# MikeIvanichev/norma

Hardware: AMD Instinct MI355X
Metric: audio-sec/wall-sec (xRT) distil-large-v3 fp16 b32 (higher is better)
Workload: dtype f16

## Files before the change

include/norma_hip.h:

```cpp
#ifndef NORMA_HIP_H
#define NORMA_HIP_H

#include <stddef.h>
#include <stdint.h>

#ifdef __cplusplus
extern "C" {
#endif

#define NH_OK 0
#define NH_ERR_INVALID 1
#define NH_ERR_HIP 2
#define NH_ERR_STATE 3
#define NH_ERR_NOMEM 4

#define NH_DTYPE_F32 0
#define NH_DTYPE_F16 1

#define NH_MAX_BATCH 96
#define NH_N_SAMPLES 480000
#define NH_N_FRAMES 3000

typedef struct nh_ctx nh_ctx;

// ... 65 lines not shown
                      float temperature, uint64_t seed, uint32_t clip0, uint32_t attempt);
int nh_detect_language(nh_ctx *ctx, const int32_t *lang_tokens, int n, int32_t *out_lang, float *out_probs);
int nh_set_languages(nh_ctx *ctx, const int32_t *langs);
int nh_transcribe_batch(nh_ctx *ctx, const float *pcm_dev, const int32_t *n_samples, int64_t stride,
                        int batch, int32_t *out_tokens, nh_decode_result *results, int max_new_tokens);
int nh_reset(nh_ctx *ctx);
int nh_synchronize(nh_ctx *ctx);

int nh_get_mel(nh_ctx *ctx, int b, float *out);
int nh_set_mel(nh_ctx *ctx, const float *mel, int batch);
int nh_encoder_output(nh_ctx *ctx, int b, float *out);
int nh_decoder_forward(nh_ctx *ctx, const int32_t *tokens, int T, float *hidden_out);
int nh_final_linear(nh_ctx *ctx, const float *x, int rows, float *logits_out);
int nh_apply_rules(nh_ctx *ctx, const float *probs, const int32_t *tokens, int n_tokens,
                   int last_timestamp, float *masked_out, int32_t *argmax_out);

int nh_sample_rules(nh_ctx *ctx, const float *probs, const int32_t *tokens, int n_tokens, int last_timestamp,
                    float temperature, uint64_t seed, uint32_t clip, uint32_t attempt, int32_t *token_out);

typedef struct nh_timings {
    float mel_ms, encoder_ms, cross_kv_ms, decode_ms;
    int32_t decode_steps;
    float gemm_ms;
    int32_t gemm_launches;
    double gemm_flops;
} nh_timings;
int nh_get_timings(nh_ctx *ctx, nh_timings *out);
int nh_set_profile_gemm(nh_ctx *ctx, int enable);

#define NH_OPT_DECODE_GRAPHS 0
#define NH_OPT_FUSE_DECODE_LAYERNORM 1
#define NH_OPT_DECODER_LAYER_LIMIT 2
#define NH_OPT_ABSORBED_XATTN 3
int nh_set_option(nh_ctx *ctx, int option, int value);

#ifdef __cplusplus
}
#endif
#endif
```

norma_amd/csrc/k_skinny.hip:

```cpp
#include <type_traits>

#include "nh_kernels.h"

__device__ __forceinline__ float gelu_tanh_d(float v) { return gelu_tanh_fast(v); }

#define SK_U 10

__device__ __forceinline__ void skinny_store(const SkinnyParams &p, f32x4 v, int r, int n, bool has_pre = false,
                                             f32x4 pre0 = (f32x4){0.f, 0.f, 0.f, 0.f}, f32x4 pre1 = (f32x4){0.f, 0.f, 0.f, 0.f}) {
    if (n >= p.N) return;
    if (has_pre) v += pre0;
    else if (p.bias) {
        if (n + 3 < p.N) v += *reinterpret_cast<const f32x4 *>(p.bias + n);
        else for (int i = 0; i < 4 && n + i < p.N; i++) v[i] += p.bias[n + i];
    }
    if (p.epi == SK_F32) {
        float *dst = reinterpret_cast<float *>(p.out[0]) + (long)r * p.ldo + n;
        if (n + 3 < p.N) *reinterpret_cast<f32x4 *>(dst) = v;
        else for (int i = 0; i < 4 && n + i < p.N; i++) dst[i] = v[i];
        return;
    }
    if (p.epi == SK_RESID_F32) {
        float *dst = reinterpret_cast<float *>(p.out[0]) + (long)r * p.ldo + n;
        f32x4 x = has_pre ? pre1 : *reinterpret_cast<const f32x4 *>(dst);
// ... 117 lines not shown
    __shared__ __attribute__((aligned(16))) float gb[2][K];
    const int tid = threadIdx.x, lane = tid & 63, w = tid >> 6;
    const int fr = lane & 15, fq = lane >> 4;
    const int tiles = (p.N + 15) >> 4, tile0 = blockIdx.x * NT;
    const int rb = blockIdx.y * 16 * NCB;
    const int kbeg = w * 32 * STEPS;
    const int wstep = p.Wt ? 512 : 32;
    half8 a[NT][STEPS];
#pragma unroll
    for (int t = 0; t < NT; t++) {
        const int tile = tile0 + t < tiles ? tile0 + t : tiles - 1;
        int wrow = tile * 16 + fr; if (wrow >= p.N) wrow = p.N - 1;
        const half_t *wp = p.Wt ? p.Wt + ((long)tile * (K >> 5) + (kbeg >> 5)) * 512 + lane * 8 : p.W + (long)wrow * K + kbeg + 8 * fq;
#pragma unroll
        for (int s = 0; s < STEPS; s++) a[t][s] = *reinterpret_cast<const half8 *>(wp + wstep * s);
    }
    f32x4 pre[NT][2];
    const bool can_pre = (p.N & 3) == 0;
#pragma unroll
    for (int t = 0; t < NT; t++) {
        pre[t][0] = (f32x4){0.f, 0.f, 0.f, 0.f}; pre[t][1] = (f32x4){0.f, 0.f, 0.f, 0.f};
        if (can_pre) {
            const int er = rb + (tid >> 2), en = (tile0 + t) * 16 + 4 * (tid & 3);
            if (tid < 64 * NCB && er < p.R && en < p.N) {
                if (p.bias) pre[t][0] = *reinterpret_cast<const f32x4 *>(p.bias + en);
                if (p.epi == SK_RESID_F32) pre[t][1] = *reinterpret_cast<const f32x4 *>(reinterpret_cast<const float *>(p.out[0]) + (long)er * p.ldo + en);
            }
        }
    }
    f32x4 xv[NCB][STEPS][2];
#pragma unroll
    for (int cb = 0; cb < NCB; cb++) {
        int r = rb + 16 * cb + fr; if (r >= p.R) r = p.R - 1;
        const float *xr = p.ln_x + (long)r * K + kbeg + 8 * fq;
#pragma unroll
        for (int s = 0; s < STEPS; s++) {
            xv[cb][s][0] = *reinterpret_cast<const f32x4 *>(xr + 32 * s);
            xv[cb][s][1] = *reinterpret_cast<const f32x4 *>(xr + 32 * s + 4);
        }
    }
    for (int c = tid; c < K / 4; c += 256) {
        reinterpret_cast<f32x4 *>(gb[0])[c] = reinterpret_cast<const f32x4 *>(p.ln_w)[c];
        reinterpret_cast<f32x4 *>(gb[1])[c] = reinterpret_cast<const f32x4 *>(p.ln_b)[c];
    }
    float mean[NCB], inv[NCB];
#pragma unroll
    for (int cb = 0; cb < NCB; cb++) {
        float s1 = 0.f;
#pragma unroll
        for (int s = 0; s < STEPS; s++) s1 = ln_sum8(s1, xv[cb][s][0], xv[cb][s][1]);
        s1 += __shfl_xor(s1, 16); s1 += __shfl_xor(s1, 32);
        if (fq == 0) part[0][w][cb][fr] = s1;
    }
    __syncthreads();
#pragma unroll
    for (int cb = 0; cb < NCB; cb++) {
        mean[cb] = ln_mean((part[0][0][cb][fr] + part[0][1][cb][fr]) + (part[0][2][cb][fr] + part[0][3][cb][fr]), p.ln_rk);
        float s2 = 0.f;
#pragma unroll
        for (int s = 0; s < STEPS; s++) s2 = ln_sq8(s2, xv[cb][s][0], xv[cb][s][1], mean[cb]);
        s2 += __shfl_xor(s2, 16); s2 += __shfl_xor(s2, 32);
        if (fq == 0) part[1][w][cb][fr] = s2;
    }
    __syncthreads();
    f32x4 acc[NT][NCB];
#pragma unroll
// ... 162 lines not shown
        if (gi == 0) {
#pragma unroll
            for (int cb = 0; cb < NCB; cb++) acc[cb] = (f32x4){0.f, 0.f, 0.f, 0.f};
        }
#pragma unroll
        for (int u = 0; u < SK_U; u++) {
            if (s0 + u < steps) {
#pragma unroll
                for (int cb = 0; cb < NCB; cb++) {
                    half8 b = *reinterpret_cast<const half8 *>(xs + (long)(s0 + u) * rows * 64 + boff[cb]);
                    acc[cb] = __builtin_amdgcn_mfma_f32_16x16x32_f16(a[u], b, acc[cb], 0, 0, 0);
                }
            }
        }
        if (gi == ngrp - 1) {
            const int n = lo + 16 * tile * tstride + 4 * fq;
            if (n < hi) {
#pragma unroll
                for (int cb = 0; cb < NCB; cb++) {
                    int r = 16 * cb + fr;
                    if (r < p.R) skinny_store(p, acc[cb], r, n);
                }
            }
        }
    };
    for (int g = 0; g < G; g += 2) {
        if (g + 1 < G) issue(g + 1, a1);
        compute(g, a0);
        if (g + 2 < G) issue(g + 2, a0);
        if (g + 1 < G) compute(g + 1, a1);
    }
}

template <int NCB>
__global__ __launch_bounds__(512) void skinny_ldsp_kernel(SkinnyParams p, int sp) {
    extern __shared__ __attribute__((aligned(16))) char xs[];
    const int tid = threadIdx.x, lane = tid & 63, w = tid >> 6;
    const int fr = lane & 15, fq = lane >> 4;
    constexpr int rows = 16 * NCB;
    const int steps = p.K >> 5;
    const int gw = blockIdx.x * 8 + w, nwav = gridDim.x * 8;
    const int ntiles = (p.N + 15) >> 4;
    const int my_tiles = gw < ntiles ? min(LP_MT, (ntiles - gw + nwav - 1) / nwav) : 0;
    int boff[NCB];
#pragma unroll
    for (int cb = 0; cb < NCB; cb++) boff[cb] = (16 * cb + fr) * 64 + ((fq ^ ((-(fr >> 2)) & 3)) << 4);
    f32x4 acc[LP_MT][NCB];
#pragma unroll
    for (int t = 0; t < LP_MT; t++)
#pragma unroll
        for (int cb = 0; cb < NCB; cb++) acc[t][cb] = (f32x4){0.f, 0.f, 0.f, 0.f};
    for (int ph0 = 0; ph0 < steps; ph0 += sp) {
        const int nst = min(sp, steps - ph0);
        const int ngrp = (nst + SK_U - 1) / SK_U;
        const int G = my_tiles * ngrp;
        auto issue = [&](int g, half8 (&a)[SK_U]) {
            const int tile = g / ngrp, s0 = ph0 + (g - tile * ngrp) * SK_U;
            const half_t *wp = p.Wt + (long)(gw + tile * nwav) * steps * 512 + lane * 8;
#pragma unroll
            for (int u = 0; u < SK_U; u++) {
                const int sc = s0 + u < steps ? s0 + u : steps - 1;
                a[u] = __builtin_nontemporal_load(reinterpret_cast<const half8 *>(wp + (long)512 * sc));
            }
        };
        half8 a0[SK_U], a1[SK_U];
        if (G > 0) issue(0, a0);
        __syncthreads();
        for (int c = tid; c < nst * rows * 4; c += 512) {
            const int q = c & 3, r = (c >> 2) % rows, st = (c >> 2) / rows;
            const int rr = r < p.R ? r : p.R - 1;
            const u32x4 v = *reinterpret_cast<const u32x4 *>(p.x + (long)rr * p.ldx + 32 * (ph0 + st) + 8 * q);
            *reinterpret_cast<u32x4 *>(xs + ((long)st * rows + r) * 64 + ((q ^ ((-(r >> 2)) & 3)) << 4)) = v;
        }
        __syncthreads();
        auto compute = [&](int g, const half8 (&a)[SK_U]) {
            const int tile = g / ngrp, s0 = (g - tile * ngrp) * SK_U;
#pragma unroll
            for (int u = 0; u < SK_U; u++) {
                if (s0 + u < nst) {
#pragma unroll
                    for (int cb = 0; cb < NCB; cb++) {
                        const half8 b = *reinterpret_cast<const half8 *>(xs + (long)(s0 + u) * rows * 64 + boff[cb]);
                        if (tile == 0) acc[0][cb] = __builtin_amdgcn_mfma_f32_16x16x32_f16(a[u], b, acc[0][cb], 0, 0, 0);
                        else acc[1][cb] = __builtin_amdgcn_mfma_f32_16x16x32_f16(a[u], b, acc[1][cb], 0, 0, 0);
                    }
                }
            }
        };
        for (int g = 0; g < G; g += 2) {
            if (g + 1 < G) issue(g + 1, a1);
            compute(g, a0);
            if (g + 2 < G) issue(g + 2, a0);
            if (g + 1 < G) compute(g + 1, a1);
        }
    }
#pragma unroll
    for (int t = 0; t < LP_MT; t++) {
        if (t < my_tiles) {
            const int n = 16 * (gw + t * nwav) + 4 * fq;
#pragma unroll
            for (int cb = 0; cb < NCB; cb++) {
                const int r = 16 * cb + fr;
                if (r < p.R) skinny_store(p, acc[t][cb], r, n);
            }
        }
    }
}

__global__ __launch_bounds__(256) void repack_tiles_kernel(const half_t *__restrict__ W, half_t *__restrict__ out, int N, int K) {
    const long chunk = blockIdx.x * 256L + threadIdx.x;
    const int steps = K >> 5;
    const long total = (long)((N + 15) >> 4) * steps * 64;
    if (chunk >= total) return;
    const int lane = (int)(chunk & 63);
    const long ts = chunk >> 6;
    const int s = (int)(ts % steps);
    const long tile = ts / steps;
    const long row = tile * 16 + (lane & 15);
    u32x4 v = {0u, 0u, 0u, 0u};
    if (row < N) v = *reinterpret_cast<const u32x4 *>(W + row * K + 32 * s + 8 * (lane >> 4));
    *reinterpret_cast<u32x4 *>(out + chunk * 8) = v;
}

void launch_repack_tiles(const half_t *W, half_t *out, int N, int K, hipStream_t st) {
    const long total = (long)((N + 15) >> 4) * (K >> 5) * 64;
    hipLaunchKernelGGL(repack_tiles_kernel, dim3((unsigned)((total + 255) / 256)), dim3(256), 0, st, W, out, N, K);
}

template <int... Vs, class F>
static void with_const(int v, F &&f) {
    (void)((v == Vs ? (f(std::integral_constant<int, Vs>{}), true) : false) || ...);
}

bool launch_skinny(const SkinnyParams &p_in, hipStream_t st) {
    const SkinnyPlan pl = skinny_plan(p_in.R, p_in.N, p_in.K, p_in.epi, p_in.Wt != nullptr, p_in.ln_x != nullptr);
    if (pl.kind == SKP_NONE) return false;
    SkinnyParams p = p_in;
    p.ln_rk = 1.0f / (float)p.K;
    const dim3 grid(pl.grid_x, pl.grid_y), block(pl.block);
    switch (pl.kind) {
        case SKP_GEMM:
            with_const<1, 2, 3, 4>(pl.ncb, [&](auto ncb) {
                constexpr int NCB = decltype(ncb)::value;
                if (pl.ksplit == 1) hipLaunchKernelGGL((skinny_gemm_kernel<NCB, 1, 2>), grid, block, 0, st, p);
                else with_const<2, 4, 8, 16>(pl.ksplit, [&](auto ks) {
                    hipLaunchKernelGGL((skinny_gemm_kernel<NCB, decltype(ks)::value, 1>), grid, block, 0, st, p);
                });
            });
            break;
        case SKP_LN:
            with_const<1, 2, 3, 4, 6, 8, 10>(pl.ksplit, [&](auto steps) {
                constexpr int STEPS = decltype(steps)::value;
                if (pl.nt == 1) hipLaunchKernelGGL((skinny_ln_kernel<STEPS, 1>), grid, block, 0, st, p);
                else hipLaunchKernelGGL((skinny_ln_kernel<STEPS, 2>), grid, block, 0, st, p);
            });
            break;
        case SKP_LDS:
            with_const<1, 2>(pl.ncb, [&](auto ncb) {
                launch_lds_exclusive<skinny_lds_kernel<decltype(ncb)::value>>(grid, block, pl.lds_used, st, p);
            });
            break;
        case SKP_LDSP:
            with_const<3, 4, 5, 6>(pl.ncb, [&](auto ncb) {
                launch_lds_exclusive<skinny_ldsp_kernel<decltype(ncb)::value>>(grid, block, pl.lds_used, st, p, pl.sp);
            });
            break;
    }
    return true;
}
```

norma_amd/csrc/nh_api.hip:

```cpp
#include <math.h>
#include <stdio.h>
#include <stdlib.h>
#include <string.h>

#include <memory>
#include <algorithm>
#include <mutex>
#include <set>
#include <string>
#include <vector>

#include "../../include/norma_hip.h"
#include "nh_kernels.h"

#define HIPCHK(expr)                                                                          \
    do {                                                                                      \
        hipError_t e_ = (expr);                                                               \
        if (e_ != hipSuccess) {                                                               \
            return ctx->fail(NH_ERR_HIP, std::string(#expr) + ": " + hipGetErrorString(e_)); \
        }                                                                                     \
    } while (0)

static thread_local std::string g_create_error;

// ... 49 lines not shown
    half_t *tok_emb_t = nullptr;
    std::vector<DecLayer> dec;
    float *pcm = nullptr;
    void *raw = nullptr; size_t raw_bytes = 0;
    int32_t *nsamp = nullptr;
    float *mel32 = nullptr;
    unsigned *chunk_max = nullptr;
    half_t *mel_img = nullptr;
    half_t *h1 = nullptr, *xn = nullptr, *q = nullptr, *k = nullptr, *vt = nullptr, *att = nullptr, *hid = nullptr,
           *xa16 = nullptr;
    float *x = nullptr, *xa32 = nullptr;
    float *dx = nullptr, *dy32 = nullptr, *logits = nullptr;
    half_t *dxn = nullptr, *dq = nullptr, *datt = nullptr, *dhid = nullptr;
    DecodeState ds{};
    uint8_t *suppress = nullptr;
    float *lpart = nullptr;
    unsigned *ltick = nullptr;
    int32_t *d_pos = nullptr;
    int pool_rows = 0, pool_max_new = 0, pool_prompt = 0;
    bool pool_per_clip_language = false;
    std::vector<char> pool_busy;
    std::vector<char> pool_held;
    std::vector<char> pool_sampled;
    std::vector<char> pool_inv_t;
    PoolSampling psamp{};
    hipGraphExec_t step_graph = nullptr;
    hipGraphExec_t multi_graph = nullptr;
    int graph_key[6] = {-1, -1, -1, -1, -1, -1};
    hipGraphExec_t step_graph_s = nullptr, multi_graph_s = nullptr;
    int graph_key_s[6] = {-1, -1, -1, -1, -1, -1};
    int token_gen = 0;
    bool opt_graphs = true, opt_fuse_ln = true;
    int opt_absorbed = 0;
    half_t *xabs_u = nullptr;
    float *xabs_z = nullptr, *xabs_ml = nullptr;
    int dec_layer_limit = 0;
    std::vector<int32_t> seq_lang;
    int32_t *d_lang_tokens = nullptr, *d_lang_out = nullptr;
    float *d_lang_probs = nullptr;
    RuleTokens tk{};
    bool have_tokens = false;
    int VP = 0;
    int32_t *h_done = nullptr;
    int cur_batch = 0, frames = 0, S = 0, last_frames = -1;
    bool have_mel = false, have_enc = false;
    hipEvent_t ev[7]{};
    nh_timings tm{};
    bool profile_gemm = false;
    std::vector<hipEvent_t> gemm_ev;
    size_t gemm_ev_used = 0;
    double gemm_flops_acc = 0.0;

    int fail(int code, const std::string &msg) { err = msg; return code; }
};

static void drop_sampled_graphs(nh_ctx *ctx) {
    if (ctx->step_graph_s) { hipGraphExecDestroy(ctx->step_graph_s); ctx->step_graph_s = nullptr; }
    if (ctx->multi_graph_s) { hipGraphExecDestroy(ctx->multi_graph_s); ctx->multi_graph_s = nullptr; }
    for (int &k : ctx->graph_key_s) k = -1;
}
static void drop_graphs(nh_ctx *ctx) {
    if (ctx->step_graph) { hipGraphExecDestroy(ctx->step_graph); ctx->step_graph = nullptr; }
    if (ctx->multi_graph) { hipGraphExecDestroy(ctx->multi_graph); ctx->multi_graph = nullptr; }
    for (int &k : ctx->graph_key) k = -1;
    drop_sampled_graphs(ctx);
}
// ... 679 lines not shown
    HIPCHK(hipGetLastError());
    ctx->have_enc = true;
    return NH_OK;
}

extern "C" int nh_encode(nh_ctx *ctx) {
    if (!ctx) return NH_ERR_INVALID;
    return encode_rows(ctx, 0, ctx->cur_batch);
}

extern "C" int nh_encode_rows(nh_ctx *ctx, int row0, int batch) {
    if (!ctx) return NH_ERR_INVALID;
    return encode_rows(ctx, row0, batch);
}

extern "C" int nh_encoder_output(nh_ctx *ctx, int b, float *out) {
    if (!ctx || !out) return NH_ERR_INVALID;
    if (!ctx->have_enc || b < 0 || b >= ctx->cur_batch) return ctx->fail(NH_ERR_STATE, "nh_encoder_output: no encoder output for that clip");
    hipSetDevice(ctx->dev);
    size_t per = (size_t)ctx->S * ctx->c.d_model;
    HIPCHK(hipMemcpyAsync(out, ctx->xa32 + per * b, per * 4, hipMemcpyDeviceToHost, ctx->st));
    HIPCHK(hipStreamSynchronize(ctx->st));
    return NH_OK;
}

#define NH_GRAPH_STEPS 8
static void skinny(nh_ctx *ctx, const half_t *x, long ldx, const LinW &W, int R, int N, int K, int epi, void *o0, void *o1,
                   void *o2, long ldo, int t0, int ctxlen, const int32_t *pos_ptr = nullptr, const float *ln_x = nullptr,
                   const float *ln_w = nullptr, const float *ln_b = nullptr) {
    SkinnyParams p{};
    p.pos_ptr = pos_ptr; p.ln_x = ln_x; p.ln_w = ln_w; p.ln_b = ln_b;
    p.x = x; p.ldx = ldx; p.W = W.w; p.Wt = W.wt; p.bias = W.b; p.R = R; p.N = N; p.K = K; p.epi = epi;
    p.out[0] = o0; p.out[1] = o1; p.out[2] = o2; p.ldo = ldo; p.d = ctx->c.d_model; p.t0 = t0; p.Tn = 1; p.ctx = ctxlen;
    if (!launch_skinny(p, ctx->sd)) {
        fprintf(stderr, "norma_hip: launch_skinny refused R=%d N=%d K=%d (ln_x %s)\n", R, N, K, ln_x ? "set" : "unset");
        abort();
    }
}

static void dec_layernorm(nh_ctx *ctx, const LnW &ln, half_t *y, float *y32, int R, int K) {
    if (!launch_layernorm_sliced(ctx->dx, ln.w, ln.b, y, y32, R, K, ctx->sd)) launch_layernorm(ctx->dx, ln.w, ln.b, y, y32, R, K, ctx->sd);
}

static void ln_skinny(nh_ctx *ctx, const LnW &ln, const LinW &W, int R, int N, int K, int epi, void *o0, void *o1, void *o2,
                      long ldo, int t0, int ctxlen, const int32_t *pos_ptr) {
    if (ctx->opt_fuse_ln && skinny_ln_supported(R, N, K)) {
        skinny(ctx, nullptr, K, W, R, N, K, epi, o0, o1, o2, ldo, t0, ctxlen, pos_ptr, ctx->dx, ln.w, ln.b);
    } else {
        dec_layernorm(ctx, ln, ctx->dxn, nullptr, R, K);
        skinny(ctx, ctx->dxn, K, W, R, N, K, epi, o0, o1, o2, ldo, t0, ctxlen, pos_ptr);
    }
}

static void decoder_step(nh_ctx *ctx, int pos, const int32_t *pos_ptr = nullptr, bool final_ln = true, bool skip_done = false) {
    const int32_t *done = skip_done ? ctx->ds.done : nullptr;
    const int d = ctx->c.d_model, B = ctx->pool_rows > 0 ? ctx->pool_rows : ctx->cur_batch, H = ctx->c.decoder_attention_heads, C = ctx->c.max_target_positions;
    launch_embed(ctx->ds.tokens, C, ctx->tok_emb, ctx->dec_pos, ctx->dx, B, 1, pos, pos_ptr, d, ctx->sd);
    int nl = 0;
    for (auto &L : ctx->dec) {
        if (ctx->dec_layer_limit > 0 && nl++ >= ctx->dec_layer_limit) break;
        ln_skinny(ctx, L.ln1, L.qkv, B, 3 * d, d, SK_QKV, ctx->dq, L.sk, L.sv, d, pos, C, pos_ptr);
        launch_dec_attention(ctx->dq, L.sk, L.sv, ctx->datt, B, 1, H, d, C, pos + 1, pos_ptr, ctx->sd, 1, done);
        skinny(ctx, ctx->datt, d, L.o, B, d, d, SK_RESID_F32, ctx->dx, nullptr, nullptr, d, 0, C);
        ln_skinny(ctx, L.ln2, L.cq, B, d, d, SK_F16, ctx->dq, nullptr, nullptr, d, 0, C, nullptr);
        if (ctx->opt_absorbed == 2) launch_xabs_attention_fast(ctx->dq, L.ckv.wt, L.ckv.w, L.ckv.b, ctx->xa16, ctx->xabs_u, ctx->xabs_z, ctx->xabs_ml, ctx->datt, B, H, d, ctx->S, done, ctx->sd);
        else if (ctx->opt_absorbed) launch_xabs_attention(ctx->dq, L.ckv.w, L.ckv.b, ctx->xa16, ctx->xabs_u, ctx->datt, B, H, d, ctx->S, done, ctx->sd);
        else launch_dec_attention(ctx->dq, L.ck, L.cv, ctx->datt, B, 1, H, d, ctx->S, ctx->S, nullptr, ctx->sd, 1, done);
        skinny(ctx, ctx->datt, d, L.co, B, d, d, SK_RESID_F32, ctx->dx, nullptr, nullptr, d, 0, C);
        ln_skinny(ctx, L.ln3, L.fc1, B, 4 * d, d, SK_GELU_F16, ctx->dhid, nullptr, nullptr, 4 * d, 0, C, nullptr);
        skinny(ctx, ctx->dhid, 4 * d, L.fc2, B, d, 4 * d, SK_RESID_F32, ctx->dx, nullptr, nullptr, d, 0, C);
    }
    if (final_ln) dec_layernorm(ctx, ctx->dec_ln, ctx->dxn, ctx->dy32, B, d);
}

static void logits_from_dx(nh_ctx *ctx, int R) {
    LinW E; E.w = ctx->tok_emb; E.wt = ctx->tok_emb_t; E.b = nullptr;
    const int d = ctx->c.d_model;
    ln_skinny(ctx, ctx->dec_ln, E, R, ctx->c.vocab_size, d, SK_F32, ctx->logits, nullptr, nullptr, ctx->VP, 0, 0, nullptr);
}

static void logits_from_dxn(nh_ctx *ctx, int R) {
    LinW E; E.w = ctx->tok_emb; E.wt = ctx->tok_emb_t; E.b = nullptr;
    skinny(ctx, ctx->dxn, ctx->c.d_model, E, R, ctx->c.vocab_size, ctx->c.d_model, SK_F32, ctx->logits, nullptr, nullptr,
           ctx->VP, 0, 0);
}

static void finish_sequence(nh_ctx *ctx, int32_t *t, int n, int done, double slp, double nsp, int32_t *out_tokens, nh_decode_result &r) {
    const int C = ctx->c.max_target_positions;
    r.no_speech_prob = nsp;
    r.no_speech_exit = (done == 2);
    if (done == 2) { r.avg_logprob = 0.0; }
    else {
        r.avg_logprob = slp / (double)n;
        while (n >= 2 && t[n - 2] > ctx->tk.no_timestamps) { t[n - 2] = t[n - 1]; n--; }
    }
    r.n_tokens = n;
    memcpy(out_tokens, t, sizeof(int32_t) * C);
    for (int i = n; i < C; i++) out_tokens[i] = 0;
}

static int capture_step_graphs(nh_ctx *ctx, int B, int max_new_tokens, int P, int mode, bool sampled = false);

static int decode_impl(nh_ctx *ctx, int32_t *out_tokens, nh_decode_result *results, int max_new_tokens, float inv_t,
                       unsigned long long seed, unsigned clip0, unsigned attempt) {
    if (!ctx || !out_tokens || !results) return ctx ? ctx->fail(NH_ERR_INVALID, "nh_decode: bad arguments") : NH_ERR_INVALID;
    if (!ctx->have_enc) return ctx->fail(NH_ERR_STATE, "nh_decode: call nh_encode first");
    if (!ctx->have_tokens) return ctx->fail(NH_ERR_STATE, "nh_decode: call nh_set_tokens first");
    if (ctx->pool_rows > 0) return ctx->fail(NH_ERR_STATE, "nh_decode: the context runs a decode pool (nh_pool_begin); a batch submitted with row0 = 0 ends it");
    hipSetDevice(ctx->dev);
    if (int rc = ensure_decoder_repack(ctx)) return rc;
// ... 422 lines not shown
    return NH_OK;
}

extern "C" int nh_set_profile_gemm(nh_ctx *ctx, int enable) {
    if (!ctx) return NH_ERR_INVALID;
    ctx->profile_gemm = enable != 0;
    return NH_OK;
}

extern "C" int nh_set_option(nh_ctx *ctx, int option, int value) {
    if (!ctx) return NH_ERR_INVALID;
    if (option == NH_OPT_DECODE_GRAPHS) ctx->opt_graphs = value != 0;
    else if (option == NH_OPT_FUSE_DECODE_LAYERNORM) { ctx->opt_fuse_ln = value != 0; drop_graphs(ctx); }
    else if (option == NH_OPT_DECODER_LAYER_LIMIT) {
        if (value < 0 || value > ctx->c.decoder_layers) return ctx->fail(NH_ERR_INVALID, "nh_set_option: layer limit outside [0, decoder_layers]");
        ctx->dec_layer_limit = value; drop_graphs(ctx);
    }
    else if (option == NH_OPT_ABSORBED_XATTN) {
        if (value < 0 || value > 2) return ctx->fail(NH_ERR_INVALID, "nh_set_option: NH_OPT_ABSORBED_XATTN takes 0, 1 or 2");
        if (value && ctx->pool_rows > 0) return ctx->fail(NH_ERR_STATE, "nh_set_option: NH_OPT_ABSORBED_XATTN covers lockstep decodes only, and the context runs a decode pool");
        if (value == 2 && !xabs_fast_supported(ctx->c.d_model, ctx->c.decoder_attention_heads)) value = 1;
        hipSetDevice(ctx->dev);
        if (value && !ctx->xabs_u) {
            ctx->xabs_u = dalloc<half_t>(ctx, (size_t)ctx->B * 32 * ctx->c.d_model);
            if (!ctx->xabs_u) return ctx->fail(NH_ERR_NOMEM, "nh_set_option: hipMalloc failed");
        }
        if (value == 2 && !ctx->xabs_z) {
            ctx->xabs_z = dalloc<float>(ctx, (size_t)ctx->B * 4 * ctx->c.decoder_attention_heads * ctx->c.d_model);
            ctx->xabs_ml = dalloc<float>(ctx, (size_t)ctx->B * 4 * 32 * 2);
            if (!ctx->xabs_z || !ctx->xabs_ml) return ctx->fail(NH_ERR_NOMEM, "nh_set_option: hipMalloc failed");
        }
        ctx->opt_absorbed = value; drop_graphs(ctx);
    }
    else return ctx->fail(NH_ERR_INVALID, "nh_set_option: unknown option " + std::to_string(option));
    return NH_OK;
}

extern "C" int nh_get_timings(nh_ctx *ctx, nh_timings *out) {
    if (!ctx || !out) return NH_ERR_INVALID;
    hipSetDevice(ctx->dev);
    HIPCHK(hipStreamSynchronize(ctx->st));
    HIPCHK(hipStreamSynchronize(ctx->sd));
    nh_timings t = ctx->tm;
    hipEventElapsedTime(&t.mel_ms, ctx->ev[0], ctx->ev[1]);
    hipEventElapsedTime(&t.encoder_ms, ctx->ev[2], ctx->ev[3]);
    hipEventElapsedTime(&t.cross_kv_ms, ctx->ev[3], ctx->ev[4]);
    hipEventElapsedTime(&t.decode_ms, ctx->ev[5], ctx->ev[6]);
    (void)hipGetLastError();
    t.gemm_ms = 0.f; t.gemm_launches = 0; t.gemm_flops = ctx->gemm_flops_acc;
    for (size_t i = 0; i + 1 < ctx->gemm_ev_used; i += 2) {
        float ms = 0.f;
        if (hipEventElapsedTime(&ms, ctx->gemm_ev[i], ctx->gemm_ev[i + 1]) == hipSuccess) { t.gemm_ms += ms; t.gemm_launches++; }
    }
    *out = t;
    return NH_OK;
}
```

norma_amd/csrc/nh_kernels.h:

```cpp
#pragma once
#include <hip/hip_runtime.h>
#include <stdint.h>

#include <atomic>

#include "skinny_plan.h"

typedef _Float16 half_t;
typedef __attribute__((ext_vector_type(8))) _Float16 half8;
typedef __attribute__((ext_vector_type(4))) _Float16 half4;
typedef __attribute__((ext_vector_type(2))) _Float16 half2v;
typedef __attribute__((ext_vector_type(2))) float f32x2;
typedef __attribute__((ext_vector_type(4))) float f32x4;
typedef __attribute__((ext_vector_type(16))) float f32x16;
typedef __attribute__((ext_vector_type(4))) unsigned int u32x4;

#define NH_MELP 128
#define NH_SP 1536
#define NH_DH 64
#define NH_MAX_DEVICES 64
#define NH_MAX_VOCAB 65536

enum GemmEpi {
    EPI_F16 = 0,
// ... 13 lines not shown
    int vt_seg;
    int head_major;
    float seg0_scale;
    int S, H;
    const float *pos;
    int cus;
    unsigned long long *dbg;
    unsigned a_magic, o_magic, s_magic;
};
static inline unsigned nh_magic(int d, long max_m) {
    if (d <= 0 || (long)d > max_m) return 0u;
    if ((unsigned long long)max_m * (unsigned long long)d >= 0x100000000ull) return ~0u;
    return (unsigned)((0x100000000ull + (unsigned)d - 1) / (unsigned)d);
}
#ifdef __HIPCC__
__device__ __forceinline__ int nh_div(int m, int d, unsigned magic) {
    return magic == 0u ? 0 : magic == ~0u ? m / d : (int)__umulhi((unsigned)m, magic);
}
#endif
void launch_gemm(const GemmParams &p, hipStream_t st);
void launch_gemm_128(const GemmParams &p, hipStream_t st);

struct SkinnyParams {
    const half_t *x; long ldx;
    const half_t *W; const float *bias;
    const half_t *Wt;
    int R, N, K;
    int epi;
    void *out[3]; long ldo;
    int d, t0, Tn, ctx;
    const int32_t *pos_ptr;
    const float *ln_x, *ln_w, *ln_b;
    float ln_rk;
};
inline bool skinny_ln_supported(int R, int N, int K) { return skinny_plan(R, N, K, SK_F32, false, true).kind != SKP_NONE; }

#ifdef __HIPCC__
__device__ __forceinline__ float gelu_tanh_fast(float v) {
#pragma clang fp contract(off)
    const float k0 = -2.0f * 0.7978845608028654f * 1.4426950408889634f;
    const float k1 = k0 * 0.044715f;
    const float m = v * __builtin_fmaf(v * v, k1, k0);
    float r = v * __builtin_amdgcn_rcpf(1.0f + __builtin_amdgcn_exp2f(m));
    asm("" : "+v"(r));
    return r;
}
__device__ __forceinline__ float ln_sum8(float acc, const f32x4 &a, const f32x4 &b) {
#pragma clang fp contract(off)
    acc += (a[0] + a[1]) + (a[2] + a[3]);
    acc += (b[0] + b[1]) + (b[2] + b[3]);
    return acc;
}
__device__ __forceinline__ float ln_sq8(float acc, const f32x4 &a, const f32x4 &b, float mean) {
#pragma clang fp contract(off)
    const f32x4 t = a - mean, u = b - mean;
    acc += __builtin_fmaf(t[1], t[1], t[0] * t[0]) + __builtin_fmaf(t[3], t[3], t[2] * t[2]);
    acc += __builtin_fmaf(u[1], u[1], u[0] * u[0]) + __builtin_fmaf(u[3], u[3], u[2] * u[2]);
    return acc;
}
__device__ __forceinline__ float ln_mean(float sum, float rk) {
#pragma clang fp contract(off)
    return sum * rk;
}
__device__ __forceinline__ float ln_inv(float sumsq, float rk) {
#pragma clang fp contract(off)
    const float var = sumsq * rk;
    return 1.0f / sqrtf(var + 1e-5f);
}
__device__ __forceinline__ f32x4 ln_apply(const f32x4 &x, float mean, float inv, const f32x4 &g, const f32x4 &b) {
#pragma clang fp contract(off)
    const f32x4 t = (x - mean) * inv;
    f32x4 o = {__builtin_fmaf(t[0], g[0], b[0]), __builtin_fmaf(t[1], g[1], b[1]), __builtin_fmaf(t[2], g[2], b[2]),
               __builtin_fmaf(t[3], g[3], b[3])};
    asm("" : "+v"(o));
    return o;
}
#endif
bool launch_layernorm_sliced(const float *x, const float *w, const float *b, half_t *y, float *y32, int M, int K, hipStream_t st);
[[nodiscard]] bool launch_skinny(const SkinnyParams &p, hipStream_t st);
void launch_repack_tiles(const half_t *W, half_t *out, int N, int K, hipStream_t st);

#define NH_LDS_EXCLUSIVE (160 * 1024)
#ifdef __HIPCC__
static inline size_t lds_exclusive_bytes(size_t needed) {
#ifdef NH_DBG_SHARE_LDS
    return needed;
#else
    (void)needed;
    return (size_t)NH_LDS_EXCLUSIVE;
#endif
}
template <auto Kernel, class... Args>
static void launch_lds_exclusive(dim3 grid, dim3 block, size_t lds_used, hipStream_t st, Args... args) {
    static std::atomic<bool> attr_set[NH_MAX_DEVICES];
    int dev = 0;
    (void)hipGetDevice(&dev);
    if (dev < 0 || dev >= NH_MAX_DEVICES || !attr_set[dev].load(std::memory_order_acquire)) {
        hipFuncSetAttribute(reinterpret_cast<const void *>(Kernel), hipFuncAttributeMaxDynamicSharedMemorySize, NH_LDS_EXCLUSIVE);
        if (dev >= 0 && dev < NH_MAX_DEVICES) attr_set[dev].store(true, std::memory_order_release);
    }
    hipLaunchKernelGGL(Kernel, grid, block, lds_exclusive_bytes(lds_used), st, args...);
}
#endif

void launch_layernorm(const float *x, const float *w, const float *b, half_t *y, float *y32, int M, int d,
                      hipStream_t st);
void launch_embed(const int32_t *tokens, int tok_stride, const half_t *E, const half_t *P, float *x, int B,
                  int Tn, int t0, const int32_t *pos_ptr, int d, hipStream_t st);

void launch_convert_samples(const void *src, float *dst, long count, int dtype, hipStream_t st);

struct MelTables {
// ... 65 lines not shown
```

norma_amd/hip.py:

```python
import ctypes as C
import os
import re
from typing import Iterable, List, Optional, Sequence, Tuple

import numpy as np

from .config import Config

_HERE = os.path.dirname(os.path.abspath(__file__))
LIB_PATH = os.environ.get("NORMA_HIP_LIB") or os.path.join(_HERE, "libnorma_hip.so")
STRICT_LIB_PATH = os.path.join(_HERE, "libnorma_hip_strict.so")
HEADER_PATH = os.path.join(os.path.dirname(_HERE), "include", "norma_hip.h")

N_SAMPLES = 480000
N_FRAMES = 3000
NH_DTYPE_F32, NH_DTYPE_F16 = 0, 1
NH_OPT_DECODE_GRAPHS, NH_OPT_FUSE_DECODE_LAYERNORM, NH_OPT_DECODER_LAYER_LIMIT, NH_OPT_ABSORBED_XATTN = 0, 1, 2, 3
SAMPLE_DTYPES = {np.dtype(np.float32): 0, np.dtype(np.float64): 1, np.dtype(np.int8): 2, np.dtype(np.int16): 3,
                 np.dtype(np.int32): 4, np.dtype(np.int64): 5, np.dtype(np.uint8): 6, np.dtype(np.uint16): 7,
                 np.dtype(np.uint32): 8, np.dtype(np.uint64): 9}


class HipError(RuntimeError):

    def __init__(self, code: int, msg: str):
        super().__init__(f"norma_hip status {code}: {msg}")
        self.code = code


class NhConfig(C.Structure):
    _fields_ = [(n, C.c_int32) for n in (
        "num_mel_bins", "max_source_positions", "d_model", "encoder_attention_heads", "encoder_layers",
        "vocab_size", "max_target_positions", "decoder_attention_heads", "decoder_layers")]


class NhTokens(C.Structure):
    _fields_ = [(n, C.c_int32) for n in
                ("sot", "eot", "lang", "task", "no_speech", "no_timestamps", "zero_sec", "one_sec")]


class NhDecodeResult(C.Structure):
    _fields_ = [("n_tokens", C.c_int32), ("no_speech_exit", C.c_int32), ("avg_logprob", C.c_double),
                ("no_speech_prob", C.c_double)]


class NhTimings(C.Structure):
    _fields_ = [("mel_ms", C.c_float), ("encoder_ms", C.c_float), ("cross_kv_ms", C.c_float),
                ("decode_ms", C.c_float), ("decode_steps", C.c_int32), ("gemm_ms", C.c_float),
                ("gemm_launches", C.c_int32), ("gemm_flops", C.c_double)]

# ... 68 lines not shown


def _fp(a):
    return a.ctypes.data_as(C.POINTER(C.c_float))


def _ip(a):
    return a.ctypes.data_as(C.POINTER(C.c_int32))


class HipWhisper:

    def __init__(self, cfg: Config, device: int = 0, max_batch: int = 1, share_with: "Optional[HipWhisper]" = None):
        self.L = load_library()
        self.cfg = cfg
        self.max_batch = max_batch
        h = C.c_void_p()
        if share_with is not None:
            rc = self.L.nh_create_shared(share_with._h, max_batch, C.byref(h))
        else:
            c = NhConfig(cfg.num_mel_bins, cfg.max_source_positions, cfg.d_model, cfg.encoder_attention_heads,
                         cfg.encoder_layers, cfg.vocab_size, cfg.max_target_positions,
                         cfg.decoder_attention_heads, cfg.decoder_layers)
            rc = self.L.nh_create(device, C.byref(c), max_batch, C.byref(h))
        if rc != 0:
            raise HipError(rc, self.L.nh_last_error(None).decode())
        self._h = h
        self.batch = 0
        self._experiment_switches()

    def _experiment_switches(self):
        if os.environ.get("NORMA_HIP_ABSORBED_XATTN"):
            self.set_option(NH_OPT_ABSORBED_XATTN, int(os.environ["NORMA_HIP_ABSORBED_XATTN"]))

    def close(self):
        if getattr(self, "_h", None):
            self.L.nh_destroy(self._h)
            self._h = None

    def __del__(self):
        try:
            self.close()
        except Exception:
            pass

    def _chk(self, rc: int):
        if rc != 0:
            raise HipError(rc, self.L.nh_last_error(self._h).decode())

    def load_tensor(self, name: str, arr: np.ndarray):
        if arr.dtype == np.float16:
            dt = NH_DTYPE_F16
        else:
            arr = np.ascontiguousarray(arr, dtype=np.float32)
            dt = NH_DTYPE_F32
        arr = np.ascontiguousarray(arr)
        shape = (C.c_int64 * arr.ndim)(*arr.shape)
        self._chk(self.L.nh_load_tensor(self._h, name.encode(), dt, shape, arr.ndim, arr.ctypes.data_as(C.c_void_p)))

    def load_weights(self, weights: Iterable[Tuple[str, np.ndarray]]):
        for name, arr in weights:
            self.load_tensor(name, arr)
        missing = self.L.nh_missing_tensors(self._h)
        if missing:
            raise HipError(3, f"{missing} tensors missing after load_weights")

# ... 196 lines not shown
```

Measured before the change: 6864.

## Fold decoder embedding into first QKV and final layernorm into logits GEMM

Adds a path where the first decoder layer's LN+QKV skinny GEMM computes the token and position embedding inline and writes dx, so the separate embed launch is skipped. Adds an LN-fused variant of the LDS-staged skinny kernel that computes final layernorm stats per row and stages normalized halves into LDS for the vocab projection when R>32. It also adds an optional interleaved tile-dealing mode. The aim is fewer decode-step launches and less global traffic, at the cost of redundant embedding and LN work across blocks and more register pressure.

```diff
diff --git a/include/norma_hip.h b/include/norma_hip.h
--- a/include/norma_hip.h
+++ b/include/norma_hip.h
@@ -121,6 +121,12 @@
 #define NH_OPT_FUSE_DECODE_LAYERNORM 1
 #define NH_OPT_DECODER_LAYER_LIMIT 2
 #define NH_OPT_ABSORBED_XATTN 3
+#define NH_OPT_FOLD_DECODE_LAUNCHES 4
+#define NH_FOLD_EMBED 1
+#define NH_FOLD_FINAL_LN 2
+#define NH_FOLD_TILE_DEAL 4
+#define NH_FOLD_ALL 7
+#define NH_FOLD_DEFAULT (NH_FOLD_EMBED | NH_FOLD_FINAL_LN)
 int nh_set_option(nh_ctx *ctx, int option, int value);
 
 #ifdef __cplusplus
diff --git a/norma_amd/csrc/k_skinny.hip b/norma_amd/csrc/k_skinny.hip
--- a/norma_amd/csrc/k_skinny.hip
+++ b/norma_amd/csrc/k_skinny.hip
@@ -173,6 +173,24 @@
 #pragma unroll
     for (int cb = 0; cb < NCB; cb++) {
         int r = rb + 16 * cb + fr; if (r >= p.R) r = p.R - 1;
+        if (p.emb_tok) {
+            const int pos = p.pos_ptr ? p.pos_ptr[r] : p.t0;
+            const int tok = p.emb_tok[(long)r * p.emb_stride + pos];
+            const half_t *er = p.emb_E + (long)tok * K + kbeg + 8 * fq, *pr = p.emb_P + (long)pos * K + kbeg + 8 * fq;
+            const bool wr = blockIdx.x == 0 && rb + 16 * cb + fr < p.R;
+            float *xo = p.emb_dx + (long)r * K + kbeg + 8 * fq;
+#pragma unroll
+            for (int s = 0; s < STEPS; s++) {
+                const half8 ev = *reinterpret_cast<const half8 *>(er + 32 * s), pv = *reinterpret_cast<const half8 *>(pr + 32 * s);
+                xv[cb][s][0] = (f32x4){(float)ev[0] + (float)pv[0], (float)ev[1] + (float)pv[1], (float)ev[2] + (float)pv[2], (float)ev[3] + (float)pv[3]};
+                xv[cb][s][1] = (f32x4){(float)ev[4] + (float)pv[4], (float)ev[5] + (float)pv[5], (float)ev[6] + (float)pv[6], (float)ev[7] + (float)pv[7]};
+                if (wr) {
+                    *reinterpret_cast<f32x4 *>(xo + 32 * s) = xv[cb][s][0];
+                    *reinterpret_cast<f32x4 *>(xo + 32 * s + 4) = xv[cb][s][1];
+                }
+            }
+            continue;
+        }
         const float *xr = p.ln_x + (long)r * K + kbeg + 8 * fq;
 #pragma unroll
         for (int s = 0; s < STEPS; s++) {
@@ -401,31 +419,33 @@
     }
 }
 
-template <int NCB>
+template <int NCB, bool LN>
 __global__ __launch_bounds__(512) void skinny_ldsp_kernel(SkinnyParams p, int sp) {
     extern __shared__ __attribute__((aligned(16))) char xs[];
     const int tid = threadIdx.x, lane = tid & 63, w = tid >> 6;
     const int fr = lane & 15, fq = lane >> 4;
     constexpr int rows = 16 * NCB;
     const int steps = p.K >> 5;
-    const int gw = blockIdx.x * 8 + w, nwav = gridDim.x * 8;
     const int ntiles = (p.N + 15) >> 4;
-    const int my_tiles = gw < ntiles ? min(LP_MT, (ntiles - gw + nwav - 1) / nwav) : 0;
+    const int tile0 = p.deal ? blockIdx.x + w * gridDim.x : blockIdx.x * 8 + w, tstep = gridDim.x * 8;
+    const int my_tiles = tile0 < ntiles ? min(LP_MT, (ntiles - tile0 + tstep - 1) / tstep) : 0;
     int boff[NCB];
 #pragma unroll
     for (int cb = 0; cb < NCB; cb++) boff[cb] = (16 * cb + fr) * 64 + ((fq ^ ((-(fr >> 2)) & 3)) << 4);
     f32x4 acc[LP_MT][NCB];
-#pragma unroll
-    for (int t = 0; t < LP_MT; t++)
-#pragma unroll
-        for (int cb = 0; cb < NCB; cb++) acc[t][cb] = (f32x4){0.f, 0.f, 0.f, 0.f};
-    for (int ph0 = 0; ph0 < steps; ph0 += sp) {
+    auto acc_zero = [&] {
+#pragma unroll
+        for (int t = 0; t < LP_MT; t++)
+#pragma unroll
+            for (int cb = 0; cb < NCB; cb++) acc[t][cb] = (f32x4){0.f, 0.f, 0.f, 0.f};
+    };
+    auto run_phase = [&](int ph0, auto &&stage) {
         const int nst = min(sp, steps - ph0);
         const int ngrp = (nst + SK_U - 1) / SK_U;
         const int G = my_tiles * ngrp;
         auto issue = [&](int g, half8 (&a)[SK_U]) {
             const int tile = g / ngrp, s0 = ph0 + (g - tile * ngrp) * SK_U;
-            const half_t *wp = p.Wt + (long)(gw + tile * nwav) * steps * 512 + lane * 8;
+            const half_t *wp = p.Wt + (long)(tile0 + tile * tstep) * steps * 512 + lane * 8;
 #pragma unroll
             for (int u = 0; u < SK_U; u++) {
                 const int sc = s0 + u < steps ? s0 + u : steps - 1;
@@ -435,12 +455,7 @@
         half8 a0[SK_U], a1[SK_U];
         if (G > 0) issue(0, a0);
         __syncthreads();
-        for (int c = tid; c < nst * rows * 4; c += 512) {
-            const int q = c & 3, r = (c >> 2) % rows, st = (c >> 2) / rows;
-            const int rr = r < p.R ? r : p.R - 1;
-            const u32x4 v = *reinterpret_cast<const u32x4 *>(p.x + (long)rr * p.ldx + 32 * (ph0 + st) + 8 * q);
-            *reinterpret_cast<u32x4 *>(xs + ((long)st * rows + r) * 64 + ((q ^ ((-(r >> 2)) & 3)) << 4)) = v;
-        }
+        stage(ph0, nst);
         __syncthreads();
         auto compute = [&](int g, const half8 (&a)[SK_U]) {
             const int tile = g / ngrp, s0 = (g - tile * ngrp) * SK_U;
@@ -462,11 +477,75 @@
             if (g + 2 < G) issue(g + 2, a0);
             if (g + 1 < G) compute(g + 1, a1);
         }
+    };
+    if constexpr (!LN) {
+        acc_zero();
+        for (int ph0 = 0; ph0 < steps; ph0 += sp)
+            run_phase(ph0, [&](int ph, int nst) {
+                for (int c = tid; c < nst * rows * 4; c += 512) {
+                    const int q = c & 3, r = (c >> 2) % rows, st = (c >> 2) / rows;
+                    const int rr = r < p.R ? r : p.R - 1;
+                    const u32x4 v = *reinterpret_cast<const u32x4 *>(p.x + (long)rr * p.ldx + 32 * (ph + st) + 8 * q);
+                    *reinterpret_cast<u32x4 *>(xs + ((long)st * rows + r) * 64 + ((q ^ ((-(r >> 2)) & 3)) << 4)) = v;
+                }
+            });
+    } else {
+        constexpr int NPASS = (NCB + 1) / 2;
+        half8 kept[NPASS][LN_MAX_STEPS / 2];
+        float *const gam = reinterpret_cast<float *>(xs + (long)sp * rows * 64), *const bet = gam + p.K;
+        const int t16 = tid & 15, n128 = p.K >> 7, k0 = (t16 >> 2) * 32 * n128 + 8 * (t16 & 3);
+        const bool upper = (t16 & 8) != 0, two = sp < steps;
+        for (int c = tid; c < p.K / 4; c += 512) {
+            reinterpret_cast<f32x4 *>(gam)[c] = reinterpret_cast<const f32x4 *>(p.ln_w)[c];
+            reinterpret_cast<f32x4 *>(bet)[c] = reinterpret_cast<const f32x4 *>(p.ln_b)[c];
+        }
+        run_phase(0, [&](int, int nst) {
+#pragma unroll
+            for (int ps = 0; ps < NPASS; ps++) {
+                const int r = (tid >> 4) + 32 * ps;
+                SlicedRow sr;
+                sliced_row_stats(sr, p.ln_x + (long)(r < p.R ? r : p.R - 1) * p.K, p.K, p.ln_rk, t16);
+#pragma unroll
+                for (int j = 0; j < LN_MAX_STEPS / 2; j++) {
+                    half8 hv[2];
+#pragma unroll
+                    for (int i = 0; i < 2; i++) {
+                        const int sI = 2 * j + i, k = k0 + 32 * (sI < n128 ? sI : 0);
+                        const f32x4 o0 = ln_apply(sr.v[sI][0], sr.mean, sr.inv, *reinterpret_cast<const f32x4 *>(gam + k), *reinterpret_cast<const f32x4 *>(bet + k));
+                        const f32x4 o1 = ln_apply(sr.v[sI][1], sr.mean, sr.inv, *reinterpret_cast<const f32x4 *>(gam + k + 4), *reinterpret_cast<const f32x4 *>(bet + k + 4));
+                        hv[i] = (half8){(half_t)o0[0], (half_t)o0[1], (half_t)o0[2], (half_t)o0[3], (half_t)o1[0], (half_t)o1[1], (half_t)o1[2], (half_t)o1[3]};
+                        const int st = k >> 5, q = (k >> 3) & 3;
+                        if (sI < n128 && st < nst && r < rows)
+                            *reinterpret_cast<half8 *>(xs + ((long)st * rows + r) * 64 + ((q ^ ((-(r >> 2)) & 3)) << 4)) = hv[i];
+                    }
+                    u32x4 o = __builtin_bit_cast(u32x4, hv[1]);
+#pragma unroll
+                    for (int c = 0; c < 4; c++) o[c] = (unsigned)__shfl_xor((int)o[c], 8);
+                    kept[ps][j] = upper ? hv[0] : __builtin_bit_cast(half8, o);
+                }
+                __builtin_amdgcn_sched_barrier(0);
+            }
+            acc_zero();
+        });
+        if (two)
+            run_phase(sp, [&](int ph, int) {
+#pragma unroll
+                for (int ps = 0; ps < NPASS; ps++) {
+                    const int r = (tid >> 4) + 32 * ps;
+#pragma unroll
+                    for (int j = 0; j < LN_MAX_STEPS / 2; j++) {
+                        const int sI = 2 * j + (upper ? 0 : 1), k = k0 + (upper ? 0 : 64 * n128) + 32 * sI;
+                        const int st = (k >> 5) - ph, q = (k >> 3) & 3;
+                        if (sI < n128 && r < rows)
+                            *reinterpret_cast<half8 *>(xs + ((long)st * rows + r) * 64 + ((q ^ ((-(r >> 2)) & 3)) << 4)) = kept[ps][j];
+                    }
+                }
+            });
     }
 #pragma unroll
     for (int t = 0; t < LP_MT; t++) {
         if (t < my_tiles) {
-            const int n = 16 * (gw + t * nwav) + 4 * fq;
+            const int n = 16 * (tile0 + t * tstep) + 4 * fq;
 #pragma unroll
             for (int cb = 0; cb < NCB; cb++) {
                 const int r = 16 * cb + fr;
@@ -502,8 +581,10 @@
 }
 
 bool launch_skinny(const SkinnyParams &p_in, hipStream_t st) {
-    const SkinnyPlan pl = skinny_plan(p_in.R, p_in.N, p_in.K, p_in.epi, p_in.Wt != nullptr, p_in.ln_x != nullptr);
+    const bool emb = p_in.emb_tok != nullptr;
+    const SkinnyPlan pl = skinny_plan(p_in.R, p_in.N, p_in.K, p_in.epi, p_in.Wt != nullptr, p_in.ln_x != nullptr || emb);
     if (pl.kind == SKP_NONE) return false;
+    if (emb && (pl.kind != SKP_LN || p_in.Tn != 1 || !p_in.emb_E || !p_in.emb_P || !p_in.emb_dx || !p_in.ln_w || !p_in.ln_b)) return false;
     SkinnyParams p = p_in;
     p.ln_rk = 1.0f / (float)p.K;
     const dim3 grid(pl.grid_x, pl.grid_y), block(pl.block);
@@ -531,9 +612,24 @@
             break;
         case SKP_LDSP:
             with_const<3, 4, 5, 6>(pl.ncb, [&](auto ncb) {
-                launch_lds_exclusive<skinny_ldsp_kernel<decltype(ncb)::value>>(grid, block, pl.lds_used, st, p, pl.sp);
+                launch_lds_exclusive<skinny_ldsp_kernel<decltype(ncb)::value, false>>(grid, block, pl.lds_used, st, p, pl.sp);
             });
             break;
     }
     return true;
 }
+
+bool launch_logits_ln(const SkinnyParams &p_in, hipStream_t st) {
+    if (!p_in.ln_x || !p_in.ln_w || !p_in.ln_b || !p_in.Wt || p_in.epi != SK_F32 || p_in.emb_tok) return false;
+    if (p_in.K % 128 != 0 || p_in.K > 128 * LN_MAX_STEPS) return false;
+    const SkinnyPlan pl = skinny_plan(p_in.R, p_in.N, p_in.K, SK_F32, true, false);
+    if (pl.kind != SKP_LDSP) return false;
+    SkinnyParams p = p_in;
+    p.ln_rk = 1.0f / (float)p.K;
+    const int steps = p.K >> 5;
+    if (pl.sp < steps && 2 * pl.sp != steps) return false;
+    with_const<3, 4, 5, 6>(pl.ncb, [&](auto ncb) {
+        launch_lds_exclusive<skinny_ldsp_kernel<decltype(ncb)::value, true>>(dim3(pl.grid_x, pl.grid_y), dim3(pl.block), pl.lds_used + (size_t)8 * p.K, st, p, pl.sp);
+    });
+    return true;
+}
diff --git a/norma_amd/csrc/nh_api.hip b/norma_amd/csrc/nh_api.hip
--- a/norma_amd/csrc/nh_api.hip
+++ b/norma_amd/csrc/nh_api.hip
@@ -105,6 +105,7 @@
     int token_gen = 0;
     bool opt_graphs = true, opt_fuse_ln = true;
     int opt_absorbed = 0;
+    int opt_fold = NH_FOLD_DEFAULT;
     half_t *xabs_u = nullptr;
     float *xabs_z = nullptr, *xabs_ml = nullptr;
     int dec_layer_limit = 0;
@@ -850,6 +851,7 @@
     p.pos_ptr = pos_ptr; p.ln_x = ln_x; p.ln_w = ln_w; p.ln_b = ln_b;
     p.x = x; p.ldx = ldx; p.W = W.w; p.Wt = W.wt; p.bias = W.b; p.R = R; p.N = N; p.K = K; p.epi = epi;
     p.out[0] = o0; p.out[1] = o1; p.out[2] = o2; p.ldo = ldo; p.d = ctx->c.d_model; p.t0 = t0; p.Tn = 1; p.ctx = ctxlen;
+    p.deal = (ctx->opt_fold & NH_FOLD_TILE_DEAL) ? 1 : 0;
     if (!launch_skinny(p, ctx->sd)) {
         fprintf(stderr, "norma_hip: launch_skinny refused R=%d N=%d K=%d (ln_x %s)\n", R, N, K, ln_x ? "set" : "unset");
         abort();
@@ -870,14 +872,29 @@
     }
 }
 
+static void embed_ln_qkv(nh_ctx *ctx, const DecLayer &L, int B, int pos, const int32_t *pos_ptr) {
+    const int d = ctx->c.d_model, C = ctx->c.max_target_positions;
+    SkinnyParams p{};
+    p.pos_ptr = pos_ptr; p.ln_w = L.ln1.w; p.ln_b = L.ln1.b;
+    p.emb_tok = ctx->ds.tokens; p.emb_stride = C; p.emb_E = ctx->tok_emb; p.emb_P = ctx->dec_pos; p.emb_dx = ctx->dx;
+    p.ldx = d; p.W = L.qkv.w; p.Wt = L.qkv.wt; p.bias = L.qkv.b; p.R = B; p.N = 3 * d; p.K = d; p.epi = SK_QKV;
+    p.out[0] = ctx->dq; p.out[1] = L.sk; p.out[2] = L.sv; p.ldo = d; p.d = d; p.t0 = pos; p.Tn = 1; p.ctx = C;
+    if (!launch_skinny(p, ctx->sd)) {
+        fprintf(stderr, "norma_hip: launch_skinny refused the embedding source R=%d d=%d\n", B, d);
+        abort();
+    }
+}
+
 static void decoder_step(nh_ctx *ctx, int pos, const int32_t *pos_ptr = nullptr, bool final_ln = true, bool skip_done = false) {
     const int32_t *done = skip_done ? ctx->ds.done : nullptr;
     const int d = ctx->c.d_model, B = ctx->pool_rows > 0 ? ctx->pool_rows : ctx->cur_batch, H = ctx->c.decoder_attention_heads, C = ctx->c.max_target_positions;
-    launch_embed(ctx->ds.tokens, C, ctx->tok_emb, ctx->dec_pos, ctx->dx, B, 1, pos, pos_ptr, d, ctx->sd);
+    const bool fold_embed = !final_ln && (ctx->opt_fold & NH_FOLD_EMBED) && ctx->opt_fuse_ln && !ctx->dec.empty() && skinny_ln_supported(B, 3 * d, d);
+    if (!fold_embed) launch_embed(ctx->ds.tokens, C, ctx->tok_emb, ctx->dec_pos, ctx->dx, B, 1, pos, pos_ptr, d, ctx->sd);
     int nl = 0;
     for (auto &L : ctx->dec) {
         if (ctx->dec_layer_limit > 0 && nl++ >= ctx->dec_layer_limit) break;
-        ln_skinny(ctx, L.ln1, L.qkv, B, 3 * d, d, SK_QKV, ctx->dq, L.sk, L.sv, d, pos, C, pos_ptr);
+        if (fold_embed && &L == &ctx->dec.front()) embed_ln_qkv(ctx, L, B, pos, pos_ptr);
+        else ln_skinny(ctx, L.ln1, L.qkv, B, 3 * d, d, SK_QKV, ctx->dq, L.sk, L.sv, d, pos, C, pos_ptr);
         launch_dec_attention(ctx->dq, L.sk, L.sv, ctx->datt, B, 1, H, d, C, pos + 1, pos_ptr, ctx->sd, 1, done);
         skinny(ctx, ctx->datt, d, L.o, B, d, d, SK_RESID_F32, ctx->dx, nullptr, nullptr, d, 0, C);
         ln_skinny(ctx, L.ln2, L.cq, B, d, d, SK_F16, ctx->dq, nullptr, nullptr, d, 0, C, nullptr);
@@ -894,6 +911,14 @@
 static void logits_from_dx(nh_ctx *ctx, int R) {
     LinW E; E.w = ctx->tok_emb; E.wt = ctx->tok_emb_t; E.b = nullptr;
     const int d = ctx->c.d_model;
+    if (R > 32 && (ctx->opt_fold & NH_FOLD_FINAL_LN) && ctx->opt_fuse_ln && E.wt) {
+        SkinnyParams p{};
+        p.ln_x = ctx->dx; p.ln_w = ctx->dec_ln.w; p.ln_b = ctx->dec_ln.b;
+        p.ldx = d; p.W = E.w; p.Wt = E.wt; p.R = R; p.N = ctx->c.vocab_size; p.K = d; p.epi = SK_F32;
+        p.out[0] = ctx->logits; p.ldo = ctx->VP; p.d = d; p.Tn = 1;
+        p.deal = (ctx->opt_fold & NH_FOLD_TILE_DEAL) ? 1 : 0;
+        if (launch_logits_ln(p, ctx->sd)) return;
+    }
     ln_skinny(ctx, ctx->dec_ln, E, R, ctx->c.vocab_size, d, SK_F32, ctx->logits, nullptr, nullptr, ctx->VP, 0, 0, nullptr);
 }
 
@@ -1382,6 +1407,10 @@
         }
         ctx->opt_absorbed = value; drop_graphs(ctx);
     }
+    else if (option == NH_OPT_FOLD_DECODE_LAUNCHES) {
+        if (value < 0 || value > NH_FOLD_ALL) return ctx->fail(NH_ERR_INVALID, "nh_set_option: NH_OPT_FOLD_DECODE_LAUNCHES takes a mask of NH_FOLD_* bits (0 .. 7)");
+        ctx->opt_fold = value; drop_graphs(ctx);
+    }
     else return ctx->fail(NH_ERR_INVALID, "nh_set_option: unknown option " + std::to_string(option));
     return NH_OK;
 }
diff --git a/norma_amd/csrc/nh_kernels.h b/norma_amd/csrc/nh_kernels.h
--- a/norma_amd/csrc/nh_kernels.h
+++ b/norma_amd/csrc/nh_kernels.h
@@ -69,6 +69,10 @@
     const int32_t *pos_ptr;
     const float *ln_x, *ln_w, *ln_b;
     float ln_rk;
+    const int32_t *emb_tok; int emb_stride;
+    const half_t *emb_E, *emb_P;
+    float *emb_dx;
+    int deal;
 };
 inline bool skinny_ln_supported(int R, int N, int K) { return skinny_plan(R, N, K, SK_F32, false, true).kind != SKP_NONE; }
 
@@ -115,6 +119,7 @@
 #endif
 bool launch_layernorm_sliced(const float *x, const float *w, const float *b, half_t *y, float *y32, int M, int K, hipStream_t st);
 [[nodiscard]] bool launch_skinny(const SkinnyParams &p, hipStream_t st);
+[[nodiscard]] bool launch_logits_ln(const SkinnyParams &p, hipStream_t st);
 void launch_repack_tiles(const half_t *W, half_t *out, int N, int K, hipStream_t st);
 
 #define NH_LDS_EXCLUSIVE (160 * 1024)
diff --git a/norma_amd/hip.py b/norma_amd/hip.py
--- a/norma_amd/hip.py
+++ b/norma_amd/hip.py
@@ -16,6 +16,9 @@
 N_FRAMES = 3000
 NH_DTYPE_F32, NH_DTYPE_F16 = 0, 1
 NH_OPT_DECODE_GRAPHS, NH_OPT_FUSE_DECODE_LAYERNORM, NH_OPT_DECODER_LAYER_LIMIT, NH_OPT_ABSORBED_XATTN = 0, 1, 2, 3
+NH_OPT_FOLD_DECODE_LAUNCHES = 4
+NH_FOLD_EMBED, NH_FOLD_FINAL_LN, NH_FOLD_TILE_DEAL, NH_FOLD_ALL = 1, 2, 4, 7
+NH_FOLD_DEFAULT = NH_FOLD_EMBED | NH_FOLD_FINAL_LN
 SAMPLE_DTYPES = {np.dtype(np.float32): 0, np.dtype(np.float64): 1, np.dtype(np.int8): 2, np.dtype(np.int16): 3,
                  np.dtype(np.int32): 4, np.dtype(np.int64): 5, np.dtype(np.uint8): 6, np.dtype(np.uint16): 7,
                  np.dtype(np.uint32): 8, np.dtype(np.uint64): 9}
@@ -150,6 +153,8 @@
     def _experiment_switches(self):
         if os.environ.get("NORMA_HIP_ABSORBED_XATTN"):
             self.set_option(NH_OPT_ABSORBED_XATTN, int(os.environ["NORMA_HIP_ABSORBED_XATTN"]))
+        if os.environ.get("NORMA_HIP_FOLD_DECODE"):
+            self.set_option(NH_OPT_FOLD_DECODE_LAUNCHES, int(os.environ["NORMA_HIP_FOLD_DECODE"]))
 
     def close(self):
         if getattr(self, "_h", None):
```

After: 6840. Within noise of the previous version (-0.4%).
